# sylvainma/Summarizer

Measured on AMD Instinct MI355X. Metric: frames scored/sec (T x 1024), higher is better.
Workload: dtype f32; 1 GPU; vasnet score, S-TVSum: 50 videos/GPU, T~U(150,320) (sum 12003), D=1024, packed batch; parallelism=video-sharded x1

## Files before the change

summarizer_amd/csrc/gemm_device.h:

```cpp
#pragma once
#include "sumk_internal.h"

namespace sumk {

typedef float f32x16 __attribute__((ext_vector_type(16)));
typedef float f32x4 __attribute__((ext_vector_type(4)));

struct GemmKArgs {
  const float* A;
  const float* B[4];
  float* C;
  const float* R;
  const float* bias0[4];
  const float* bias1[4];
  const GemmProb* probs;
  int32_t nprob;
  int32_t n_group;
  int32_t total_tiles;
  Drop drop; uint32_t drop_site;
  int32_t xcd_tiles_m;
  int32_t group_remap;
  float alpha;
  int32_t lean;
  float* moments;
  unsigned short* C16;
  const float* ln_stats; const float* ln_c1; const float* ln_c2;
  int32_t sk_epi; float* sk_part; unsigned* sk_cnt; float* Csel[4];
};

typedef const __attribute__((address_space(4))) int64_t* cptr64;
typedef const __attribute__((address_space(4))) int32_t* cptr32;
__device__ __forceinline__ int prob_tile_start(const GemmProb* p, int i) { return ((cptr32)(uintptr_t)(p + i))[15]; }
__device__ __forceinline__ GemmProb load_prob(const GemmProb* p, int i) {
  const cptr64 q = (cptr64)(uintptr_t)(p + i);
  const cptr32 r = (cptr32)(uintptr_t)(p + i);
  GemmProb P;
  P.a_off = q[0]; P.b_off = q[1]; P.c_off = q[2]; P.r_off = q[3];
  P.M = r[8]; P.N = r[9]; P.K = r[10]; P.lda = r[11]; P.ldb = r[12]; P.ldc = r[13]; P.ldr = r[14];
  P.tile_start = r[15]; P.tiles_n = r[16];
  return P;
}
static_assert(offsetof(GemmProb, M) == 32 && offsetof(GemmProb, tile_start) == 60 && offsetof(GemmProb, tiles_n) == 64, "GemmProb layout");

struct TileCtx {
  int64_t c_off, r_off;
  int32_t M, N, K, lda, ldb, ldc, ldr, m0, n0, klast;
  const float* ab; const float* bb;
};

template <int BM, int BN>
// ... 90 lines not shown
          if (ka.drop.thr) v = drop_apply(ka.drop, ka.drop_site, (uint64_t)row * (uint64_t)cur.N + (uint64_t)col, v);
          v += ka.R[cur.r_off + (int64_t)row * cur.ldr + col];
        }
        if constexpr (EPI == EPI_ACCUM) v = *cp + ka.alpha * v;
        if constexpr (EPI == EPI_NONE) {
          if (ka.C) *cp = v;
          if (ka.C16) ka.C16[cur.c_off + (int64_t)row * cur.ldc + col] = __builtin_bit_cast(unsigned short, (__bf16)v);
        } else {
          *cp = v;
        }
      }
    }
  }
}

__device__ __forceinline__ float dpp_row_sum16(float v) {
  v += __builtin_bit_cast(float, __builtin_amdgcn_update_dpp(0, __builtin_bit_cast(int, v), 0xB1, 0xF, 0xF, true));
  v += __builtin_bit_cast(float, __builtin_amdgcn_update_dpp(0, __builtin_bit_cast(int, v), 0x4E, 0xF, 0xF, true));
  v += __builtin_bit_cast(float, __builtin_amdgcn_update_dpp(0, __builtin_bit_cast(int, v), 0x141, 0xF, 0xF, true));
  v += __builtin_bit_cast(float, __builtin_amdgcn_update_dpp(0, __builtin_bit_cast(int, v), 0x140, 0xF, 0xF, true));
  return v;
}

template <int TM, int TN>
__device__ __forceinline__ void epilogue_head_moments(const GemmKArgs& ka, const TileCtx& cur, const f32x16 (&acc)[TM][TN], int row0,
                                                      int col0, int li, int lh, float2* lds_stats, int m0, int tid) {
  static_assert(TN == 2, "head epilogue: a wave covers one 64-column slot");
  float bias[TN], gw[TN], c1[TN];
  bool colok[TN];
  const bool ln = ka.ln_stats != nullptr;
  if (ln) {
    __syncthreads();
    if (tid < 128) lds_stats[tid] = reinterpret_cast<const float2*>(ka.ln_stats)[min(m0 + tid, cur.M - 1)];
    __syncthreads();
  }
#pragma unroll
  for (int tn = 0; tn < TN; ++tn) {
    const int col = col0 + tn * 32 + li;
    colok[tn] = col < cur.N;
    const int cc = colok[tn] ? col : 0;
    bias[tn] = ka.bias0[0][cc];
    gw[tn] = ka.bias1[0][cc] * ka.bias1[1][cc];
    c1[tn] = 0.f;
    if (ln) { c1[tn] = ka.ln_c1[cc]; bias[tn] += ka.ln_c2[cc]; }
  }
  const int slots = cur.N >> 5, slot = (col0 >> 5) + (li >> 4);
  float4* part = reinterpret_cast<float4*>(ka.C);
#pragma unroll
  for (int tm = 0; tm < TM; ++tm) {
#pragma unroll
    for (int r = 0; r < 16; ++r) {
      float s1 = 0.f, s2 = 0.f, s3 = 0.f;
      float mean = 0.f, rstd = 1.f;
      if (ln) {
        const float2 st = lds_stats[row0 - m0 + tm * 32 + (r & 3) + 8 * (r >> 2) + 4 * lh];
        mean = st.x; rstd = st.y;
      }
#pragma unroll
      for (int tn = 0; tn < TN; ++tn) {
        float v = rstd * (acc[tm][tn][r] - mean * c1[tn]) + bias[tn];
        v = (v < 0.f) ? 0.f : v;
        if (!colok[tn]) v = 0.f;
        s1 += v; s2 += v * v; s3 += v * gw[tn];
      }
      s1 = dpp_row_sum16(s1); s2 = dpp_row_sum16(s2); s3 = dpp_row_sum16(s3);
      const int row = row0 + tm * 32 + (r & 3) + 8 * (r >> 2) + 4 * lh;
      if ((li & 15) == 0 && row < cur.M) part[(int64_t)row * slots + slot] = make_float4(s1, s2, s3, 0.f);
    }
  }
}

template <int TM, int TN>
__device__ __forceinline__ void epilogue_row_moments(const GemmKArgs& ka, const TileCtx& cur, const f32x16 (&acc)[TM][TN], int row0,
                                                     int col0, int li, int lh) {
  static_assert(TN == 1 || TN == 2, "moments epilogue: a wave covers 32 or 64 columns");
  bool colok[TN];
#pragma unroll
  for (int tn = 0; tn < TN; ++tn) colok[tn] = col0 + tn * 32 + li < cur.N;
  const int slots = TN == 2 ? cur.N >> 5 : cur.N >> 4, slot = (TN == 2 ? col0 >> 5 : col0 >> 4) + (li >> 4);
  float2* part = reinterpret_cast<float2*>(ka.moments) + (cur.c_off / cur.ldc) * slots;
#pragma unroll
  for (int tm = 0; tm < TM; ++tm) {
#pragma unroll
    for (int r = 0; r < 16; ++r) {
      float s1 = 0.f, s2 = 0.f;
#pragma unroll
      for (int tn = 0; tn < TN; ++tn) {
        const float v = colok[tn] ? acc[tm][tn][r] : 0.f;
        s1 += v; s2 += v * v;
      }
      s1 = dpp_row_sum16(s1); s2 = dpp_row_sum16(s2);
      const int row = row0 + tm * 32 + (r & 3) + 8 * (r >> 2) + 4 * lh;
      if ((li & 15) == 0 && row < cur.M) part[(int64_t)row * slots + slot] = make_float2(s1, s2);
    }
// ... 26 lines not shown
```

summarizer_amd/csrc/gemm_f32.hip:

```cpp
#include "gemm_regstage.h"

namespace sumk {

int launch_gemm(GemmLayout layout, GemmEpi epi, const GemmLaunch& g, hipStream_t stream) {
  SUMK_ARG(g.A && g.B[0] && (g.C || (g.C16 && epi == EPI_NONE)) && g.probs, "gemm: null operand");
  if (g.total_tiles <= 0) return SUMK_OK;
  GemmKArgs ka;
  ka.A = g.A;
  for (int i = 0; i < 4; ++i) { ka.B[i] = g.B[i]; ka.bias0[i] = g.bias0[i]; ka.bias1[i] = g.bias1[i]; }
  ka.C = g.C; ka.R = g.R; ka.probs = g.probs; ka.nprob = g.nprob; ka.n_group = g.n_group; ka.alpha = g.alpha;
  ka.total_tiles = g.total_tiles; ka.xcd_tiles_m = 0;
  const bool small_groups = (int64_t)g.total_tiles <= (int64_t)256 * g.nprob;
  ka.group_remap = (g.nprob > 1 && (g.group_remap || (g.precision != SUMK_PRECISION_FP32 && small_groups))) ? 1 : 0;
  ka.drop.seed = g.drop_seed; ka.drop.thr = g.drop_thr; ka.drop.scale = g.drop_scale; ka.drop.seed_dev = nullptr; ka.drop_site = g.drop_site;
  ka.lean = (g.lean && g.nprob == 1 && layout == GEMM_NT && g.small_tile == 0 && g.precision == SUMK_PRECISION_FP32 &&
             (g.n_group == 0 || g.n_group % 128 == 0)) ? 1 : 0;
  ka.C16 = (unsigned short*)g.C16;
  SUMK_ARG(!g.C16 || epi == EPI_NONE, "gemm: the bf16 copy of C goes with the plain epilogue");
  SUMK_ARG(!g.src16 || (g.small_tile == 0 && g.n_group == 0), "gemm: bf16-source launches use 128x128 tiles and one B operand");
  ka.moments = g.moments; ka.ln_stats = g.ln_stats; ka.ln_c1 = g.ln_c1; ka.ln_c2 = g.ln_c2;
  SUMK_ARG(epi != EPI_RESIDUAL_MOMENTS || g.moments, "gemm: the moments epilogue needs an output buffer");
  SUMK_ARG(!g.ln_stats || (epi == EPI_BIAS_RELU_HEAD && g.ln_c1 && g.ln_c2), "gemm: ln_stats goes with the head epilogue and c1 / c2");
  if (g.prof_tag >= 0) prof_begin(g.prof_tag, stream);
  prof_begin(SUMK_PROF_GEMM_ALL, stream);
  if (g.nprob == 1 && g.xcd_M > 0) {
    const int bm = (g.src16 && g.wide16) ? g.wide16 : gemm_tile_m(g.small_tile), bn = (g.src16 && g.wide16) ? 256 : gemm_tile_n(g.small_tile);
    const int tm = (g.xcd_M + bm - 1) / bm, tn = (g.xcd_N + bn - 1) / bn;
    if (tn % 4 == 0 && tm >= 16) { ka.xcd_tiles_m = tm; ka.total_tiles = 8 * ((tm + 1) / 2) * (tn / 4); }
  }
  int rc;
  ka.sk_epi = (int32_t)epi; ka.sk_part = g.sk_part; ka.sk_cnt = g.sk_cnt;
  for (int i = 0; i < 4; ++i) ka.Csel[i] = g.Csel[i];
  if (g.sk) {
    SUMK_ARG(g.precision == SUMK_PRECISION_FP32 && g.small_tile == 1 && g.n_group == 0 && !g.src16 && !g.C16 && g.C,
             "gemm: an SK launch is exact fp32 on 64x64 tiles with one B group per table entry");
    SUMK_ARG(epi == EPI_NONE || epi == EPI_RESIDUAL || epi == EPI_BIAS_RELU || epi == EPI_ACCUM, "gemm: epilogue %d has no SK form", (int)epi);
    SUMK_ARG(g.drop_thr == 0, "gemm: SK launches have no epilogue dropout");
    ka.group_remap = 0; ka.xcd_tiles_m = 0;
    rc = launch_gemm_lean(layout, ka, ka.total_tiles, stream, 1);
    prof_end(SUMK_PROF_GEMM_ALL, stream);
    if (g.prof_tag >= 0) prof_end(g.prof_tag, stream);
    if (rc != SUMK_OK) return rc;
    SUMK_HIP(hipGetLastError());
    return SUMK_OK;
  }
// ... 356 lines not shown
```

summarizer_amd/csrc/gemm_regstage.h:

```cpp
#pragma once
#include "gemm_device.h"
#include <algorithm>
#include <cstdlib>

namespace sumk {

typedef __bf16 bf16x4 __attribute__((ext_vector_type(4)));
typedef __bf16 bf16x8 __attribute__((ext_vector_type(8)));
typedef short s16x4 __attribute__((ext_vector_type(4)));
typedef short s16x8 __attribute__((ext_vector_type(8)));

__device__ __forceinline__ float4 ldg4(const float* p) { return *reinterpret_cast<const float4*>(p); }

__device__ __forceinline__ bf16x8 tr_frag(const char* p, int pitch) {
  typedef __attribute__((address_space(3))) s16x4* lds_s16x4;
  const s16x4 h0 = __builtin_amdgcn_ds_read_tr16_b64_v4i16((lds_s16x4)(p));
  const s16x4 h1 = __builtin_amdgcn_ds_read_tr16_b64_v4i16((lds_s16x4)(p + 4 * pitch));
  return __builtin_bit_cast(bf16x8, __builtin_shufflevector(h0, h1, 0, 1, 2, 3, 4, 5, 6, 7));
}

template <int BM, int BN, int BK, bool A_KC, bool B_KC, int EPI, int NS = 0, bool LEAN = false>
__global__ __launch_bounds__(256, 3) void gemm_f32_kernel(GemmKArgs ka) {
  static_assert(!LEAN || (A_KC && B_KC && NS == 0), "LEAN: NT fp32 instances only");
  constexpr bool X3 = NS > 0;
  static_assert(NS >= 0 && NS <= 3, "operand split: 0 (fp32), 1 (plain bf16), 2 or 3 bf16 planes");
  constexpr int KC_PITCH = (NS == 0 ? BK : NS * BK / 2) + 4;
  constexpr int TPK = BK / 4, RPP = 256 / TPK;
  constexpr int WTM = BM / 2, WTN = BN / 2;
  constexpr int TM = WTM / 32, TN = WTN / 32;
  constexpr int NLDA = BM * BK / 1024, NLDB = BN * BK / 1024;
  constexpr int MCP_A = 2 * BM + 64, MCP_B = 2 * BN + 64;
  constexpr int A_ELEMS = A_KC ? BM * KC_PITCH : (X3 ? NS * BK * MCP_A / 4 : BK * BM);
  constexpr int B_ELEMS = B_KC ? BN * KC_PITCH : (X3 ? NS * BK * MCP_B / 4 : BK * BN);
  constexpr int STAGE = A_ELEMS + B_ELEMS;
  __shared__ __attribute__((aligned(16))) float lds[STAGE];
  float* sA = lds;
  float* sB = lds + A_ELEMS;

  const int tid = threadIdx.x;
  const int lane = tid & 63;
  const int wave = tid >> 6;
  const int wm = wave >> 1, wn = wave & 1;
  const int li = lane & 31, lh = lane >> 5;
  constexpr int TPRA = BM / 4, TPRB = BN / 4;
  constexpr int KROWSA = 256 / TPRA, KROWSB = 256 / TPRB;
  const int kq4 = (tid % TPK) * 4;

  const float* pa[NLDA];
  const float* pb[NLDB];
  int voa[NLDA], vob[NLDB];

  auto setup = [&](int tile, TileCtx& c) -> bool {
    GemmProb P;
    if (!decode_tile<BM, BN>(ka, tile, c, P)) return false;
    if constexpr (LEAN) {
      c.ab = ka.A + P.a_off;
      int g = 0, ng = 0;
      if (ka.n_group > 0) { g = c.n0 / ka.n_group; ng = g * ka.n_group; }
// ... 201 lines not shown
            float4 v = *reinterpret_cast<const float4*>(&sB[(wn * WTN + t * 32 + li) * KC_PITCH + kk * 8 + 4 * lh]);
            bv[t][0] = v.x; bv[t][1] = v.y; bv[t][2] = v.z; bv[t][3] = v.w;
          } else {
#pragma unroll
            for (int j = 0; j < 4; ++j) bv[t][j] = sB[(kk * 8 + 4 * lh + j) * BN + wn * WTN + t * 32 + li];
          }
        }
#pragma unroll
        for (int j = 0; j < 4; ++j)
#pragma unroll
          for (int tm = 0; tm < TM; ++tm)
#pragma unroll
            for (int tn = 0; tn < TN; ++tn)
              acc[tm][tn] = __builtin_amdgcn_mfma_f32_32x32x2f32(av[tm][j], bv[tn][j], acc[tm][tn], 0, 0, 0);
      }
      }
  };

  int tile = blockIdx.x;
  if (tile >= ka.total_tiles) return;
  TileCtx cur, nxt;
  if (!setup(tile, cur)) return;
  gload(cur, 0);

  while (true) {
    f32x16 acc[TM][TN];
    if constexpr (EPI == EPI_RESIDUAL || EPI == EPI_RESIDUAL_MOMENTS) {
      residual_init<TM, TN>(ka, cur, acc, cur.m0 + wm * WTM, cur.n0 + wn * WTN, li, lh);
    } else {
#pragma unroll
      for (int i = 0; i < TM; ++i)
#pragma unroll
        for (int j = 0; j < TN; ++j)
#pragma unroll
          for (int r = 0; r < 16; ++r) acc[i][j][r] = 0.f;
    }

    const int next_tile = tile + gridDim.x;
    bool has_next = false;
    const int K = cur.K;
    {
      int k0 = 0;
      for (; k0 + BK < K; k0 += BK) {
        __syncthreads();
        swrite(sA, sB);
        __syncthreads();
        gload(cur, k0 + BK);
        compute(sA, sB, acc);
      }
      __syncthreads();
      ktail(K, k0);
      swrite(sA, sB);
      __syncthreads();
      has_next = next_tile < ka.total_tiles;
      if (has_next) has_next = setup(next_tile, nxt);
      if (has_next) gload(nxt, 0);
      compute(sA, sB, acc);
    }

    if constexpr (EPI == EPI_BIAS_RELU_HEAD) {
      epilogue_head_moments<TM, TN>(ka, cur, acc, cur.m0 + wm * WTM, cur.n0 + wn * WTN, li, lh, reinterpret_cast<float2*>(lds), cur.m0, tid);
    } else if constexpr (EPI == EPI_RESIDUAL_MOMENTS) {
      epilogue_row_moments<TM, TN>(ka, cur, acc, cur.m0 + wm * WTM, cur.n0 + wn * WTN, li, lh);
      epilogue_store<EPI, TM, TN, true>(ka, cur, acc, cur.m0 + wm * WTM, cur.n0 + wn * WTN, li, lh);
    } else {
      epilogue_store<EPI, TM, TN, true>(ka, cur, acc, cur.m0 + wm * WTM, cur.n0 + wn * WTN, li, lh);
    }
    if (!has_next) break;
    tile = next_tile;
    cur = nxt;
  }
}

template <int BM, int BN, int BK, bool A_KC, bool B_KC, int X3 = 0>
static int launch_epi(GemmEpi epi, const GemmKArgs& ka, int tiles, hipStream_t s) {
  constexpr int occ = (BM == 128 && BN == 128) ? 3 : (BM == 128 ? 4 : (BK == 64 ? 4 : 8));
  dim3 grid(std::min(tiles, 256 * occ)), block(256);
  if constexpr (BM == 128 && BN == 128 && BK == 32 && A_KC && B_KC && X3 == 0) {
    if (ka.lean) {
#define SUMK_LEAN_CASE(E) case E: hipLaunchKernelGGL((gemm_f32_kernel<BM, BN, BK, true, true, E, 0, true>), grid, block, 0, s, ka); return SUMK_OK;
      switch (epi) {
        SUMK_LEAN_CASE(EPI_NONE) SUMK_LEAN_CASE(EPI_RESIDUAL) SUMK_LEAN_CASE(EPI_BIAS_RELU) SUMK_LEAN_CASE(EPI_BIAS2)
        SUMK_LEAN_CASE(EPI_BIAS_RESIDUAL) SUMK_LEAN_CASE(EPI_BIAS_RELU_HEAD) SUMK_LEAN_CASE(EPI_RESIDUAL_MOMENTS)
        default: break;
      }
#undef SUMK_LEAN_CASE
    }
  }
  switch (epi) {
    case EPI_NONE: hipLaunchKernelGGL((gemm_f32_kernel<BM, BN, BK, A_KC, B_KC, EPI_NONE, X3>), grid, block, 0, s, ka); break;
    case EPI_RESIDUAL: hipLaunchKernelGGL((gemm_f32_kernel<BM, BN, BK, A_KC, B_KC, EPI_RESIDUAL, X3>), grid, block, 0, s, ka); break;
    case EPI_BIAS_RELU: hipLaunchKernelGGL((gemm_f32_kernel<BM, BN, BK, A_KC, B_KC, EPI_BIAS_RELU, X3>), grid, block, 0, s, ka); break;
    case EPI_BIAS2: hipLaunchKernelGGL((gemm_f32_kernel<BM, BN, BK, A_KC, B_KC, EPI_BIAS2, X3>), grid, block, 0, s, ka); break;
    case EPI_ACCUM: hipLaunchKernelGGL((gemm_f32_kernel<BM, BN, BK, A_KC, B_KC, EPI_ACCUM, X3>), grid, block, 0, s, ka); break;
    case EPI_BIAS_RESIDUAL: hipLaunchKernelGGL((gemm_f32_kernel<BM, BN, BK, A_KC, B_KC, EPI_BIAS_RESIDUAL, X3>), grid, block, 0, s, ka); break;
    case EPI_BIAS_RELU_HEAD:
      if constexpr (BM == 128 && BN == 128 && BK == 32 && A_KC && B_KC) {
        hipLaunchKernelGGL((gemm_f32_kernel<BM, BN, BK, A_KC, B_KC, EPI_BIAS_RELU_HEAD, X3>), grid, block, 0, s, ka); break;
      } else { set_error("gemm: the head epilogue exists for 128x128 NT tiles only"); return SUMK_ERR_ARG; }
    case EPI_RESIDUAL_MOMENTS:
      if constexpr ((BM == 128 && BN == 128 && BK == 32 && A_KC && B_KC) || (BM == 64 && BN == 64 && BK == 32 && A_KC && !B_KC)) {
        hipLaunchKernelGGL((gemm_f32_kernel<BM, BN, BK, A_KC, B_KC, EPI_RESIDUAL_MOMENTS, X3>), grid, block, 0, s, ka); break;
      } else { set_error("gemm: the moments epilogue exists for 128x128 NT and 64x64 NN tiles only"); return SUMK_ERR_ARG; }
    default: set_error("gemm: bad epilogue %d", (int)epi); return SUMK_ERR_ARG;
  }
  return SUMK_OK;
}

template <int BM, int BN, int BK, int X3 = 0>
static int launch_layout(GemmLayout layout, GemmEpi epi, const GemmKArgs& ka, int tiles, hipStream_t s) {
  if (layout == GEMM_NT) return launch_epi<BM, BN, BK, true, true, X3>(epi, ka, tiles, s);
  if (layout == GEMM_NN) return launch_epi<BM, BN, BK, true, false, X3>(epi, ka, tiles, s);
  return launch_epi<BM, BN, BK, false, false, X3>(epi, ka, tiles, s);
}


}
```

summarizer_amd/csrc/sumk_internal.h:

```cpp
#pragma once
#include <hip/hip_runtime.h>
#include <stdint.h>
#include <stddef.h>
#include "../../include/sumk.h"

namespace sumk {

void set_error(const char* fmt, ...);
int hip_fail(hipError_t e, const char* what);

#define SUMK_HIP(call)                                             \
  do {                                                             \
    hipError_t _e = (call);                                        \
    if (_e != hipSuccess) return ::sumk::hip_fail(_e, #call);      \
  } while (0)
#define SUMK_ARG(cond, ...)                                        \
  do {                                                             \
    if (!(cond)) { ::sumk::set_error(__VA_ARGS__); return SUMK_ERR_ARG; } \
  } while (0)
#define SUMK_TRY(call)                                             \
  do { int _r = (call); if (_r != SUMK_OK) return _r; } while (0)

inline size_t align_up(size_t v, size_t a) { return (v + a - 1) / a * a; }


struct GemmProb {
  int64_t a_off, b_off, c_off, r_off;
  int32_t M, N, K;
  int32_t lda, ldb, ldc, ldr;
  int32_t tile_start;
  int32_t tiles_n;
  int32_t pad_[7];
};
static_assert(sizeof(GemmProb) == 96, "GemmProb layout");
enum { SK_N = 0, SK_IDX = 1, SK_TILE0 = 2, SK_BSEL = 3, SK_CSEL = 4, SK_PART0 = 5 };

enum GemmLayout { GEMM_NT = 0, GEMM_NN = 1, GEMM_TN = 2 };
enum GemmEpi {
  EPI_NONE = 0,
  EPI_RESIDUAL = 1,
  EPI_BIAS_RELU = 2,
  EPI_BIAS2 = 3,
  EPI_ACCUM = 4,
  EPI_BIAS_RESIDUAL = 5,
  EPI_BIAS_RELU_HEAD = 6,
  EPI_RESIDUAL_MOMENTS = 7,
};

struct GemmLaunch {
  const float* A = nullptr;
  const float* B[4] = {nullptr, nullptr, nullptr, nullptr};
  float* C = nullptr;
  const float* R = nullptr;
  const float* bias0[4] = {nullptr, nullptr, nullptr, nullptr};
  const float* bias1[4] = {nullptr, nullptr, nullptr, nullptr};
  const GemmProb* probs = nullptr;
  int32_t nprob = 1;
  int32_t n_group = 0;
  int32_t total_tiles = 0;
  float alpha = 1.f;
  int32_t small_tile = 0;
  int32_t prof_tag = -1;
  int32_t precision = 0;
  int32_t xcd_M = 0, xcd_N = 0;
  int32_t no_dma = 0;
  uint64_t drop_seed = 0; uint32_t drop_thr = 0, drop_site = 0; float drop_scale = 1.f;
  float* moments = nullptr;
  int32_t lean = 0;
  int32_t src16 = 0;
  int32_t wide16 = 0;
  void* C16 = nullptr;
  int32_t group_remap = 0;
  const float* ln_stats = nullptr; const float* ln_c1 = nullptr; const float* ln_c2 = nullptr;
  int32_t sk = 0; float* sk_part = nullptr; unsigned* sk_cnt = nullptr; float* Csel[4] = {nullptr, nullptr, nullptr, nullptr};
};
constexpr int SK_MAX_SLICES = 8;
inline int sk_slices(int tiles, int K, int* kchunk) {
  int S = tiles > 0 ? 1024 / tiles : 1;
  S = S < 1 ? 1 : S > SK_MAX_SLICES ? SK_MAX_SLICES : S;
  if (S > K / 128) S = K / 128 < 1 ? 1 : K / 128;
  int kc = ((K + S - 1) / S + 31) / 32 * 32;
  S = (K + kc - 1) / kc;
  *kchunk = kc;
  return S;
}

inline int gemm_tile_m(int cfg) { return cfg == 1 ? 64 : 128; }
inline int gemm_tile_n(int cfg) { return cfg == 0 ? 128 : cfg == 3 ? 256 : 64; }
inline int gemm_tile_dim(int cfg) { return gemm_tile_n(cfg); }
inline int gemm_tiles(int M, int N, int cfg) {
  int tm = gemm_tile_m(cfg), tn = gemm_tile_n(cfg);
  return ((M + tm - 1) / tm) * ((N + tn - 1) / tn);
}
int launch_gemm(GemmLayout layout, GemmEpi epi, const GemmLaunch& g, hipStream_t stream);
inline int gemm_b16_ok(int64_t M, int64_t N, int64_t K, int lda, int ldb, bool kc_a, bool kc_b) {
  const int64_t lim = (int64_t)1 << 31;
// ... 165 lines not shown
```

summarizer_amd/csrc/vasnet.hip:

```cpp
#include "gemm_device.h"
#include <math.h>
#include <algorithm>
#include <cstdlib>

namespace sumk {

enum { TB_S = 0, TB_PV = 1, TB_DV = 2, TB_DP = 3, TB_DQ = 4, TB_DK = 5, TB_COUNT = 6 };
constexpr int ROW_PROBS = 8;
constexpr int SPLITK_PROBS = 64;
constexpr int COLSUM_CHUNKS = 128;

struct VasnetWs {
  size_t qkv, e, ctx, y0, y1, z, seq, prob_row, prob_seq, prob_dvk, prob_skw, stats, scores, row_seq, total;
  size_t total_core;
  size_t e2, dz, dy1, dy0, dctx, dqkv, lnpart, colpart, slab, prob_sk;
  size_t x16, w16, ctx16, y116, dz16, dy016, dqkv16, qkv16, dctx16, p16, s16;
  size_t slab_elems;
  int64_t e_elems;
  int32_t n_rows;
  size_t sk_part, sk_cnt, sk_tabs, sk_part_bytes;
  size_t tab_bytes;
};

constexpr int SK_MAX_ROWS = 1024;
// ... 699 lines not shown
    for (int k = sub; k < slots; k += 8) { const float2 p = moments[(int64_t)row * slots + k]; s1 += p.x; s2 += p.y; }
#pragma unroll
  for (int m = 1; m <= 4; m <<= 1) { s1 += __shfl_xor(s1, m, 64); s2 += __shfl_xor(s2, m, 64); }
  if (row >= n_rows || sub != 0) return;
  const double mean = s1 / D, var = s2 / D - mean * mean;
  stats[row] = make_float2((float)mean, (float)(1.0 / sqrt((var > 0.0 ? var : 0.0) + (double)eps)));
}
__global__ void head_vectors_kernel(const float* __restrict__ b1, const float* __restrict__ c2, const float* __restrict__ ln_w,
                                    const float* __restrict__ w2, int D, float* __restrict__ biasc, float* __restrict__ gw) {
  const int n = blockIdx.x * blockDim.x + threadIdx.x;
  if (n < D) { biasc[n] = b1[n] + c2[n]; gw[n] = ln_w[n] * w2[n]; }
}

struct WPlanes { size_t wqkv, wo, w1g, c1, biasc, gw, tmp, total; };
static WPlanes wplanes_layout(int D, int np) {
  WPlanes l; size_t p = 0;
  auto take = [&](size_t bytes) { size_t at = p; p += align_up(bytes, 256); return at; };
  l.wqkv = take(pw_planes_bytes(3 * (int64_t)D, D, np)); l.wo = take(pw_planes_bytes(D, D, np)); l.w1g = take(pw_planes_bytes(D, D, np));
  l.c1 = take((size_t)D * 4); l.biasc = take((size_t)D * 4); l.gw = take((size_t)D * 4);
  l.tmp = take((size_t)D * D * 4 + (size_t)D * 4);
  l.total = p;
  return l;
}
struct PwExtra { size_t qkv, ap, ctx, total; };
static PwExtra pw_extra(int D, int64_t R, int t_max, int np, size_t base) {
  PwExtra e; size_t p = align_up(base, 256);
  auto take = [&](size_t bytes) { size_t at = p; p += align_up(bytes, 256); return at; };
  e.qkv = take(pw_planes_bytes(R, 3 * D, np)); e.ap = take(pw_alpha_bytes(R, t_max, np)); e.ctx = take(pw_planes_bytes(R, D, np));
  e.total = p;
  return e;
}
constexpr int PW_LONG_TMIN = 1536;
struct PwLong { size_t e, qp, kp, vt, ap, st, qk, total; int tn, kpad, qk_direct; };
static PwLong pw_long_layout(int D, int64_t R, int t_max, int np, size_t base) {
  PwLong e; size_t p = align_up(base, 256);
  auto take = [&](size_t bytes) { size_t at = p; p += align_up(bytes, 256); return at; };
  e.tn = (t_max + 255) / 256 * 256; e.kpad = (t_max + 31) / 32 * 32;
  e.e = take((size_t)t_max * e.tn * 4);
  e.qk_direct = (R >= e.tn && pw_ok(R, 2 * (int64_t)D, D, R, 3 * (int64_t)D, np) && (int64_t)pw_planes_bytes(R, 2 * D, np) < (((int64_t)1 << 31) - 65536)) ? 1 : 0;
  e.qk = take(e.qk_direct ? pw_planes_bytes(R, 2 * D, np) : 0);
  e.qp = take(e.qk_direct ? 0 : pw_planes_bytes(e.tn, D, np)); e.kp = take(e.qk_direct ? 0 : pw_planes_bytes(e.tn, D, np));
  e.vt = take(pw_planes_bytes(D, e.kpad, np)); e.ap = take(pw_planes_bytes(t_max, e.kpad, np));
  e.st = take((size_t)t_max * 8);
  e.total = p;
  return e;
}
// ... 419 lines not shown
  float* none[4] = {nullptr, nullptr, nullptr, nullptr};
  SUMK_TRY(gemm_tn_splitk_accum_multi(2, As, Bs, D, D, D, D, R, nullptr, L.slab_elems, pskw, SPLITK_PROBS, none, D, D, 1.f, stream, precision, b16, SPLITK_TABLE_ONLY));
  SUMK_TRY(gemm_tn_splitk_accum((const float*)base, 3 * D, (const float*)base, D, 3 * D, D, R, nullptr, L.slab_elems, pskw + SPLITK_PROBS, SPLITK_PROBS, none, D, D, 1.f,
                                stream, precision, b16, SPLITK_TABLE_ONLY));
  return SUMK_OK;
}

extern "C" int sumk_vasnet_build_tables(int32_t D, int32_t n_seq, const int32_t* seq_off_host, const int32_t* seq_off_dev, int32_t training,
                                        int32_t precision, void* tables, size_t tables_bytes, void* stream_) {
  hipStream_t stream = (hipStream_t)stream_;
  SUMK_ARG(seq_off_dev && tables && ((uintptr_t)tables & 255) == 0, "vasnet_build_tables: null or misaligned (256 B) pointer");
  SUMK_ARG(precision >= SUMK_PRECISION_FP32 && precision <= SUMK_PRECISION_MAX, "vasnet_build_tables: unknown precision %d", precision);
  Geometry G;
  SUMK_TRY(geometry(D, n_seq, seq_off_host, training, precision, 0, &G));
  if (tables_bytes < G.L.tab_bytes) { set_error("vasnet_build_tables: %zu bytes < required %zu", tables_bytes, G.L.tab_bytes); return SUMK_ERR_WORKSPACE; }
  launch_setup(G, D, n_seq, seq_off_dev, (char*)tables, stream);
  if (G.sk) SUMK_TRY(launch_sk_setup(G, D, n_seq, seq_off_dev, (char*)tables, stream));
  if (training) SUMK_TRY(build_skw_tables(G, D, (GemmProb*)((char*)tables + G.L.prob_skw), precision, stream));
  SUMK_HIP(hipGetLastError());
  return SUMK_OK;
}

extern "C" size_t sumk_vasnet_wplanes_bytes(int32_t D, int32_t n_planes) {
  return wplanes_ok(D, n_planes) ? wplanes_layout(D, n_planes).total : 0;
}

extern "C" int sumk_vasnet_wplanes_build(int32_t D, const sumk_vasnet_weights* w, const float* Wvo, int32_t n_planes, void* out, size_t out_bytes,
                                         void* stream_) {
  hipStream_t stream = (hipStream_t)stream_;
  SUMK_ARG(wplanes_ok(D, n_planes), "vasnet_wplanes_build: D=%d planes=%d is not eligible (D %% 256, 2 or 3 planes)", D, n_planes);
  SUMK_ARG(w && w->Wk && w->Wq && w->Wv && w->Wo && w->W1 && w->b1 && w->w2 && w->ln_w && w->ln_b && out, "vasnet_wplanes_build: null pointer");
  const WPlanes l = wplanes_layout(D, n_planes);
  SUMK_ARG(out_bytes >= l.total && ((uintptr_t)out & 255) == 0, "vasnet_wplanes_build: buffer of %zu bytes (256-byte aligned) needed, got %zu", l.total, out_bytes);
  char* o = (char*)out;
  SUMK_HIP(hipMemsetAsync(o, 0, l.c1, stream));
  const float* parts[3] = {w->Wq, w->Wk, Wvo ? Wvo : w->Wv};
  for (int i = 0; i < 3; ++i) SUMK_TRY(split_planes_at(parts[i], D, D, D, n_planes, o + l.wqkv, (int64_t)i * D, 3 * (int64_t)D, stream));
  SUMK_TRY(split_planes(w->Wo, D, D, D, n_planes, o + l.wo, stream));
  float* W1g = (float*)(o + l.tmp); float* c2 = W1g + (size_t)D * D;
  hipLaunchKernelGGL(ln_fold_stats_kernel, dim3(D), dim3(256), 0, stream, w->W1, w->ln_w, w->ln_b, D, W1g, (float*)(o + l.c1), c2,
                     (const float2*)nullptr, 0, 0, 0.f, (float2*)nullptr);
  SUMK_HIP(hipGetLastError());
  SUMK_TRY(split_planes(W1g, D, D, D, n_planes, o + l.w1g, stream));
  hipLaunchKernelGGL(head_vectors_kernel, dim3((D + 255) / 256), dim3(256), 0, stream, w->b1, c2, w->ln_w, w->w2, D, (float*)(o + l.biasc), (float*)(o + l.gw));
  SUMK_HIP(hipGetLastError());
  return SUMK_OK;
}

extern "C" size_t sumk_vasnet_workspace_bytes(int32_t D, int32_t n_seq, const int32_t* seq_off_host, int32_t training) {
  VasnetWs w;
  if (carve(D, n_seq, seq_off_host, training, &w) != SUMK_OK) return 0;
  return w.total;
// ... 236 lines not shown
    const dim3 sg((R + 3) / 4), sb(256);
    float* e2p = use_e2 ? E2 : nullptr;
    unsigned short* p16 = b16 ? (unsigned short*)(ws + L.p16) : nullptr;
#define SUMK_SOFTMAX(NR) hipLaunchKernelGGL(vasnet_softmax_kernel<NR>, sg, sb, 0, stream, E, e2p, seq, (const int32_t*)(tb + L.row_seq), n_seq, R, opts->scale, opts->ignore_self, opts->aperture, drop, p16, (const float*)E, 0, (int64_t)0)
    if (t_max <= 256) SUMK_SOFTMAX(4); else if (t_max <= 512) SUMK_SOFTMAX(8); else if (t_max <= 1024) SUMK_SOFTMAX(16); else SUMK_SOFTMAX(0);
#undef SUMK_SOFTMAX
  }
  }
  static const bool fused_head_on = !(getenv("SUMK_FUSED_HEAD") && getenv("SUMK_FUSED_HEAD")[0] == '0');
  static const bool fused_ln_on = !(getenv("SUMK_FUSED_LN") && getenv("SUMK_FUSED_LN")[0] == '0');
  const bool fused_tail = fused_head_on && !training && drop.thr == 0 && G.st_d == 0 && D % 64 == 0;
  const int ln_slots = Wvo ? D / 16 : D / 32;
  const size_t ln_mom_f = align_up((size_t)R * ln_slots * 2, 64), ln_w_f = (size_t)D * D, ln_c_f = align_up((size_t)2 * D, 64);
  const bool fused_ln = pw || (fused_tail && fused_ln_on && (!Wvo || G.cfg_pv == 1) && ln_mom_f + ln_w_f + ln_c_f + (size_t)2 * R <= (size_t)R * D);
  char* const pw_ctxp = pw_attn ? ws + px.ctx : ws + L.y0;
  char* const pw_y0p = (pw_attn && Wvo) ? ws + px.ctx : pw_attn ? ws + px.qkv : ws + L.qkv;
  float* const pw_mom = Z;
  float* const pw_stats = Z + align_up((size_t)R * (D / 16) * 2, 64);
  float* const pw_part = pw_stats + align_up((size_t)R * 2, 64);
  float* ln_moments = pw ? pw_mom : Y1;
  float* ln_W1g = Y1 + ln_mom_f;
  float* ln_c1 = ln_W1g + ln_w_f;
  float* ln_stats = ln_c1 + ln_c_f;
  if (!G.attn_fused && !pw_attn && !pw_long) {
    GemmLaunch g; g.precision = opts->precision;
    g.A = use_e2 ? E2 : E; g.B[0] = QKV; g.C = Wvo ? Y0 : CTX; g.R = x; g.probs = tabs + TB_PV * n_seq; g.nprob = n_seq; g.small_tile = G.cfg_pv;
    g.total_tiles = G.tiles_pv; g.prof_tag = SUMK_PROF_GEMM_PV;
    if (Wvo && fused_ln) g.moments = ln_moments;
    if (b16) { g.A = (const float*)(ws + L.p16); g.B[0] = (const float*)(ws + L.qkv16); g.src16 = 1; g.C16 = ws + L.ctx16; g.C = nullptr; }
    SUMK_TRY(launch_gemm(GEMM_NN, Wvo ? (fused_ln ? EPI_RESIDUAL_MOMENTS : EPI_RESIDUAL) : EPI_NONE, g, stream));
    if (Wvo && pw) {
      hipLaunchKernelGGL(ln_row_stats_kernel, dim3((R + 31) / 32), dim3(256), 0, stream, (const float2*)pw_mom, ln_slots, R, D, opts->eps, (float2*)pw_stats);
      SUMK_HIP(hipGetLastError());
      SUMK_TRY(split_planes(Y0, R, D, D, np, pw_y0p, stream));
    } else
    if (Wvo && fused_ln) {
      hipLaunchKernelGGL(ln_fold_stats_kernel, dim3(D + (R + 31) / 32), dim3(256), 0, stream, w->W1, w->ln_w, w->ln_b, D, ln_W1g, ln_c1,
                         ln_c1 + D, (const float2*)ln_moments, ln_slots, R, opts->eps, (float2*)ln_stats);
      SUMK_HIP(hipGetLastError());
    }
  }
  if (pw_attn && Wvo) {
    hipLaunchKernelGGL(ln_row_stats_kernel, dim3((R + 31) / 32), dim3(256), 0, stream, (const float2*)pw_mom, D / 32, R, D, opts->eps, (float2*)pw_stats);
    SUMK_HIP(hipGetLastError());
  } else
  if (pw && !Wvo) {
    if (!pw_attn && !pw_long) SUMK_TRY(split_planes(CTX, R, D, D, np, pw_ctxp, stream));
    PwLaunch g; g.A = pw_ctxp; g.a_rows = R; g.B = wp + wl.wo; g.b_rows = D; g.M = R; g.N = D; g.K = D; g.np = np;
    g.R = x; g.ldr = D; g.moments = pw_mom; g.O = pw_y0p; g.o_rows = R; g.prof_tag = SUMK_PROF_GEMM_OPROJ;
    SUMK_TRY(launch_gemm_pw(PW_RES_MOM_PLANES, g, stream));
    hipLaunchKernelGGL(ln_row_stats_kernel, dim3((R + 31) / 32), dim3(256), 0, stream, (const float2*)pw_mom, D / 64, R, D, opts->eps, (float2*)pw_stats);
    SUMK_HIP(hipGetLastError());
  } else
  if (!Wvo) {
    GemmLaunch g; g.precision = opts->precision;
    g.A = CTX; g.B[0] = w->Wo; g.C = Y0; g.R = x; g.probs = prow + RP_DD; g.small_tile = G.st_d;
    g.total_tiles = gemm_tiles(R, D, G.st_d); g.xcd_M = R; g.xcd_N = D; g.prof_tag = SUMK_PROF_GEMM_OPROJ;
    g.lean = lean_rows;
    if (fused_ln) {
      g.moments = ln_moments;
      SUMK_TRY(launch_gemm(GEMM_NT, EPI_RESIDUAL_MOMENTS, g, stream));
      hipLaunchKernelGGL(ln_fold_stats_kernel, dim3(D + (R + 31) / 32), dim3(256), 0, stream, w->W1, w->ln_w, w->ln_b, D, ln_W1g, ln_c1,
                         ln_c1 + D, (const float2*)ln_moments, ln_slots, R, opts->eps, (float2*)ln_stats);
      SUMK_HIP(hipGetLastError());
    } else {
      if (b16) to_b16(g, ws + L.ctx16, Wo16, R, D, prow, RP_DD_W);
      SUMK_TRY(launch_gemm(GEMM_NT, EPI_RESIDUAL, g, stream));
    }
  }
  if (!fused_ln) launch_ln_rows<false>(Y0, b16 ? nullptr : Y1, w->ln_w, w->ln_b, nullptr, nullptr, nullptr, R, D, opts->eps, stats, drop, 1u, stream,
                                       b16 ? (unsigned short*)(ws + L.y116) : nullptr);
  if (pw) {
    PwLaunch g; g.A = pw_y0p; g.a_rows = R; g.B = wp + wl.w1g; g.b_rows = D; g.M = R; g.N = D; g.K = D; g.np = np;
    g.bias = (const float*)(wp + wl.biasc); g.gw = (const float*)(wp + wl.gw); g.ln_c1 = (const float*)(wp + wl.c1); g.ln_stats = pw_stats;
    g.head_part = pw_part; g.prof_tag = SUMK_PROF_GEMM_K1;
    SUMK_TRY(launch_gemm_pw(PW_HEAD, g, stream));
    hipLaunchKernelGGL(head_finalize_kernel, dim3((R + 31) / 32), dim3(256), 0, stream, (const float4*)pw_part, D / 64, R, D, w->ln_w,
                       w->ln_b, w->w2, w->b2, opts->eps, scores);
    SUMK_HIP(hipGetLastError());
    return SUMK_OK;
  }
  if (fused_tail) {
    GemmLaunch g; g.precision = opts->precision;
    g.A = Y1; g.B[0] = w->W1; g.bias0[0] = w->b1; g.bias1[0] = w->ln_w; g.bias1[1] = w->w2;
    if (fused_ln) { g.A = Y0; g.B[0] = ln_W1g; g.ln_stats = ln_stats; g.ln_c1 = ln_c1; g.ln_c2 = ln_c1 + D; }
    g.C = Z;
    g.probs = prow + RP_DD; g.small_tile = 0;
    g.total_tiles = gemm_tiles(R, D, 0); g.xcd_M = R; g.xcd_N = D; g.prof_tag = SUMK_PROF_GEMM_K1;
    g.lean = lean_rows;
    SUMK_TRY(launch_gemm(GEMM_NT, EPI_BIAS_RELU_HEAD, g, stream));
    hipLaunchKernelGGL(head_finalize_kernel, dim3((R + 31) / 32), dim3(256), 0, stream, (const float4*)Z, D / 32, R, D, w->ln_w,
                       w->ln_b, w->w2, w->b2, opts->eps, scores);
    SUMK_HIP(hipGetLastError());
    return SUMK_OK;
  }
  {
    GemmLaunch g; g.precision = opts->precision;
    g.A = Y1; g.B[0] = w->W1; g.bias0[0] = w->b1; g.C = Z; g.probs = prow + RP_DD; g.small_tile = G.st_d;
    g.total_tiles = gemm_tiles(R, D, G.st_d); g.xcd_M = R; g.xcd_N = D; g.prof_tag = SUMK_PROF_GEMM_K1;
    g.lean = lean_rows;
    if (b16) to_b16(g, ws + L.y116, W116, R, D, prow, RP_DD_W);
    SUMK_TRY(launch_gemm(GEMM_NT, EPI_BIAS_RELU, g, stream));
  }
  launch_ln_rows<true>(Z, training ? (float*)(ws + L.scores) : nullptr, w->ln_w, w->ln_b, w->w2, w->b2, scores, R, D, opts->eps, stats ? stats + 2 * (size_t)R : nullptr, drop, 2u, stream);
  SUMK_HIP(hipGetLastError());
  return SUMK_OK;
}

extern "C" int sumk_vasnet_forward(float* x, int32_t D, int32_t n_seq, const int32_t* seq_off_host,
                                   const int32_t* seq_off_dev, const sumk_vasnet_weights* w,
                                   const sumk_vasnet_opts* opts, const float* pos_table, const int32_t* pos_rows,
                                   float* scores, void* workspace, size_t workspace_bytes, int32_t training,
                                   void* stream) {
// ... 240 lines not shown
```

summarizer_amd/models/vasnet.py:

```python
import math
import random
import numpy as np
import torch
import torch.nn as nn
import torch.nn.init as init

from .. import kernels
from ..autograd import SegmentMseMeanFunction
from . import Trainer
from ._positional import PositionalInput, _sinusoid_table, packed_pos_input
from ..training import FlatAdam, dist_info, plan_shards, resolve_batch_videos, step_video_total


class VASNet(PositionalInput, nn.Module):
    def __init__(self, input_size=1024, max_length=None, pos_embed="simple", ignore_self=False,
                 attention_aperture=None, scale=None, epsilon=1e-6, weight_init="xavier", precision="fp32", fold_vo=False):
        super().__init__()
        self.precision = precision
        self.fold_vo = bool(fold_vo)
        self._wvo, self._wvo_key = None, None
        self.input_size = input_size
        self.aperture = attention_aperture
        self.ignore_self = ignore_self
        self.scale = scale if scale is not None else 1 / np.sqrt(self.input_size)
# ... 43 lines not shown

    def score_packed(self, x_packed, lens):
        sb = kernels.SeqBatch.get(lens, x_packed.device)
        if self.max_length is None:
            return self._score(x_packed, sb, None, None)
        plane_path = self.precision in kernels.PLANES_OF and self.input_size % 256 == 0 and sb.n_rows >= 256
        xp, extra = packed_pos_input(self, x_packed, sb, self.precision, kernels.PLANES_OF[self.precision] if plane_path else 0)
        return self._score(xp, sb, None, None, extra)

    def _score(self, xp, sb, table, rows, extra=None):
        training = self.training and torch.is_grad_enabled()
        if training or (torch.is_grad_enabled() and any(p.requires_grad for p in self.parameters())):
            from ..autograd import VasnetFunction
            names = [k for _, k in kernels.VASNET_FIELDS]
            p = self._params()
            opts = self._opts(self.training)
            opts.update(extra or {})
            return VasnetFunction.apply(xp, sb, opts, table, rows, names, *[p[n] for n in names])
        opts = self._opts(False)
        opts.update(extra or {})
        wvo = self._folded() if self.fold_vo else None
        if self.precision in kernels.PLANES_OF and table is None and self.input_size % 256 == 0 and sb.n_rows >= 256:
            opts["wplanes"] = self._wplanes(wvo)
        scores, _ = kernels.vasnet_forward_packed(xp, sb, self._params(), opts, table, rows, training=False, wvo=wvo)
        return scores

    def _wplanes(self, wvo):
        p = self._params()
        key = kernels.weights_key([v for _, v in sorted(p.items())], self.precision, bool(self.fold_vo))
        return kernels.cached_block(self, "_wpl", key, lambda out: kernels.vasnet_wplanes(
            {k: v.detach() for k, v in p.items()}, self.input_size, kernels.PLANES_OF[self.precision], wvo=wvo, out=out))

    def _folded(self):
        wo, wv = self.attention_head_projection.weight, self.V.weight
        key = (wo.data_ptr(), wv.data_ptr(), wo._version, wv._version, kernels.WEIGHTS_EPOCH[0])
        if self._wvo is None or self._wvo_key != key:
            with torch.no_grad():
                self._wvo = kernels.fold_vo(wo.detach(), wv.detach(), out=self._wvo if self._wvo is not None and self._wvo.device == wo.device else None)
            self._wvo_key = key
        return self._wvo

    def _drop_weight_caches(self):
        self._wvo_key = None
        self._wpl_key = None

    def invalidate_folded(self):
        self._drop_weight_caches()

    def train(self, mode=True):
        self._drop_weight_caches()
        return super().train(mode)

    def load_state_dict(self, *args, **kwargs):
        self._drop_weight_caches()
# ... 127 lines not shown
```

Measured before the change: 10.49 million frames/s.

## Compute LN row statistics inside the head GEMM and cache the folded W1 weights

Adds a head epilogue variant where each 128x128 tile reduces the per-row moment partials into mean and rstd in shared memory, using double accumulation, right after its first loads are issued. This removes the separate ln_fold_stats launch for fp32 inference. The gamma-folded W1 and the c1/c2 vectors are now built once into a cached weights block keyed on weight versions, so they are no longer recomputed on every forward. In exchange, each column tile re-reads the row moments redundantly, adds two extra barriers per tile, and needs more LDS.

```diff
diff --git a/summarizer_amd/csrc/gemm_device.h b/summarizer_amd/csrc/gemm_device.h
--- a/summarizer_amd/csrc/gemm_device.h
+++ b/summarizer_amd/csrc/gemm_device.h
@@ -26,6 +26,7 @@
   unsigned short* C16;
   const float* ln_stats; const float* ln_c1; const float* ln_c2;
   int32_t sk_epi; float* sk_part; unsigned* sk_cnt; float* Csel[4];
+  const float* ln_moments_in; int32_t ln_slots; float ln_eps;
 };
 
 typedef const __attribute__((address_space(4))) int64_t* cptr64;
@@ -162,14 +163,14 @@
   return v;
 }
 
-template <int TM, int TN>
+template <int TM, int TN, bool STATS_READY = false>
 __device__ __forceinline__ void epilogue_head_moments(const GemmKArgs& ka, const TileCtx& cur, const f32x16 (&acc)[TM][TN], int row0,
                                                       int col0, int li, int lh, float2* lds_stats, int m0, int tid) {
   static_assert(TN == 2, "head epilogue: a wave covers one 64-column slot");
   float bias[TN], gw[TN], c1[TN];
   bool colok[TN];
-  const bool ln = ka.ln_stats != nullptr;
-  if (ln) {
+  const bool ln = STATS_READY || ka.ln_stats != nullptr;
+  if (ln && !STATS_READY) {
     __syncthreads();
     if (tid < 128) lds_stats[tid] = reinterpret_cast<const float2*>(ka.ln_stats)[min(m0 + tid, cur.M - 1)];
     __syncthreads();
@@ -210,6 +211,51 @@
   }
 }
 
+__device__ __forceinline__ void head_row_stats(const GemmKArgs& ka, const TileCtx& cur, float* lds, float2* lds_stats, int tid) {
+  const float2* mom = reinterpret_cast<const float2*>(ka.ln_moments_in);
+  int K = cur.K; float eps = ka.ln_eps;
+  asm volatile("" : "+v"(tid), "+s"(K), "+s"(eps));
+  const int slots = ka.ln_slots, sub = tid & 7, rl0 = tid >> 3;
+  double* sums = reinterpret_cast<double*>(lds);
+  __syncthreads();
+  constexpr int NK = 4;
+  if (slots <= 8 * NK) {
+    float2 q[4][NK];
+#pragma unroll
+    for (int p = 0; p < 4; ++p) {
+      const int row = min(cur.m0 + p * 32 + rl0, cur.M - 1);
+#pragma unroll
+      for (int u = 0; u < NK; ++u) q[p][u] = sub + 8 * u < slots ? mom[(int64_t)row * slots + sub + 8 * u] : make_float2(0.f, 0.f);
+    }
+#pragma unroll
+    for (int p = 0; p < 4; ++p) {
+      double s1 = 0.0, s2 = 0.0;
+#pragma unroll
+      for (int u = 0; u < NK; ++u)
+        if (sub + 8 * u < slots) { s1 += q[p][u].x; s2 += q[p][u].y; }
+#pragma unroll
+      for (int m = 1; m <= 4; m <<= 1) { s1 += __shfl_xor(s1, m, 64); s2 += __shfl_xor(s2, m, 64); }
+      if (sub == 0) { sums[2 * (p * 32 + rl0)] = s1; sums[2 * (p * 32 + rl0) + 1] = s2; }
+    }
+  } else {
+#pragma unroll 1
+    for (int p = 0; p < 4; ++p) {
+      const int row = min(cur.m0 + p * 32 + rl0, cur.M - 1);
+      double s1 = 0.0, s2 = 0.0;
+      for (int k = sub; k < slots; k += 8) { const float2 q = mom[(int64_t)row * slots + k]; s1 += q.x; s2 += q.y; }
+#pragma unroll
+      for (int m = 1; m <= 4; m <<= 1) { s1 += __shfl_xor(s1, m, 64); s2 += __shfl_xor(s2, m, 64); }
+      if (sub == 0) { sums[2 * (p * 32 + rl0)] = s1; sums[2 * (p * 32 + rl0) + 1] = s2; }
+    }
+  }
+  __syncthreads();
+  if (tid < 128) {
+    const double s1 = sums[2 * tid], s2 = sums[2 * tid + 1];
+    const double mean = s1 / K, var = s2 / K - mean * mean;
+    lds_stats[tid] = make_float2((float)mean, (float)(1.0 / sqrt((var > 0.0 ? var : 0.0) + (double)eps)));
+  }
+}
+
 template <int TM, int TN>
 __device__ __forceinline__ void epilogue_row_moments(const GemmKArgs& ka, const TileCtx& cur, const f32x16 (&acc)[TM][TN], int row0,
                                                      int col0, int li, int lh) {
diff --git a/summarizer_amd/csrc/gemm_f32.hip b/summarizer_amd/csrc/gemm_f32.hip
--- a/summarizer_amd/csrc/gemm_f32.hip
+++ b/summarizer_amd/csrc/gemm_f32.hip
@@ -21,6 +21,9 @@
   ka.moments = g.moments; ka.ln_stats = g.ln_stats; ka.ln_c1 = g.ln_c1; ka.ln_c2 = g.ln_c2;
   SUMK_ARG(epi != EPI_RESIDUAL_MOMENTS || g.moments, "gemm: the moments epilogue needs an output buffer");
   SUMK_ARG(!g.ln_stats || (epi == EPI_BIAS_RELU_HEAD && g.ln_c1 && g.ln_c2), "gemm: ln_stats goes with the head epilogue and c1 / c2");
+  ka.ln_moments_in = g.ln_moments_in; ka.ln_slots = g.ln_slots; ka.ln_eps = g.ln_eps;
+  SUMK_ARG(epi != EPI_BIAS_RELU_HEAD_ROWS || (g.ln_moments_in && g.ln_slots > 0 && g.ln_c1 && g.ln_c2 && ka.lean && !g.src16 && !g.sk),
+           "gemm: the head epilogue with in-launch row statistics is one exact-fp32 NT problem on the buffer-load 128x128 instance, with moments and c1 / c2");
   if (g.prof_tag >= 0) prof_begin(g.prof_tag, stream);
   prof_begin(SUMK_PROF_GEMM_ALL, stream);
   if (g.nprob == 1 && g.xcd_M > 0) {
diff --git a/summarizer_amd/csrc/gemm_regstage.h b/summarizer_amd/csrc/gemm_regstage.h
--- a/summarizer_amd/csrc/gemm_regstage.h
+++ b/summarizer_amd/csrc/gemm_regstage.h
@@ -33,7 +33,9 @@
   constexpr int A_ELEMS = A_KC ? BM * KC_PITCH : (X3 ? NS * BK * MCP_A / 4 : BK * BM);
   constexpr int B_ELEMS = B_KC ? BN * KC_PITCH : (X3 ? NS * BK * MCP_B / 4 : BK * BN);
   constexpr int STAGE = A_ELEMS + B_ELEMS;
-  __shared__ __attribute__((aligned(16))) float lds[STAGE];
+  constexpr bool HEAD_ROWS = EPI == EPI_BIAS_RELU_HEAD_ROWS;
+  static_assert(!HEAD_ROWS || (BM == 128 && BN == 128 && A_KC && B_KC && NS == 0 && LEAN), "in-launch row statistics: the exact-fp32 buffer-load instance on 128x128 NT tiles");
+  __shared__ __attribute__((aligned(16))) float lds[STAGE + (HEAD_ROWS ? 256 : 0)];
   float* sA = lds;
   float* sB = lds + A_ELEMS;
 
@@ -281,6 +283,7 @@
   TileCtx cur, nxt;
   if (!setup(tile, cur)) return;
   gload(cur, 0);
+  if constexpr (HEAD_ROWS) head_row_stats(ka, cur, lds, reinterpret_cast<float2*>(lds + STAGE), tid);
 
   while (true) {
     f32x16 acc[TM][TN];
@@ -317,7 +320,9 @@
       compute(sA, sB, acc);
     }
 
-    if constexpr (EPI == EPI_BIAS_RELU_HEAD) {
+    if constexpr (HEAD_ROWS) {
+      epilogue_head_moments<TM, TN, true>(ka, cur, acc, cur.m0 + wm * WTM, cur.n0 + wn * WTN, li, lh, reinterpret_cast<float2*>(lds + STAGE), cur.m0, tid);
+    } else if constexpr (EPI == EPI_BIAS_RELU_HEAD) {
       epilogue_head_moments<TM, TN>(ka, cur, acc, cur.m0 + wm * WTM, cur.n0 + wn * WTN, li, lh, reinterpret_cast<float2*>(lds), cur.m0, tid);
     } else if constexpr (EPI == EPI_RESIDUAL_MOMENTS) {
       epilogue_row_moments<TM, TN>(ka, cur, acc, cur.m0 + wm * WTM, cur.n0 + wn * WTN, li, lh);
@@ -328,6 +333,7 @@
     if (!has_next) break;
     tile = next_tile;
     cur = nxt;
+    if constexpr (HEAD_ROWS) head_row_stats(ka, cur, lds, reinterpret_cast<float2*>(lds + STAGE), tid);
   }
 }
 
@@ -341,6 +347,7 @@
       switch (epi) {
         SUMK_LEAN_CASE(EPI_NONE) SUMK_LEAN_CASE(EPI_RESIDUAL) SUMK_LEAN_CASE(EPI_BIAS_RELU) SUMK_LEAN_CASE(EPI_BIAS2)
         SUMK_LEAN_CASE(EPI_BIAS_RESIDUAL) SUMK_LEAN_CASE(EPI_BIAS_RELU_HEAD) SUMK_LEAN_CASE(EPI_RESIDUAL_MOMENTS)
+        SUMK_LEAN_CASE(EPI_BIAS_RELU_HEAD_ROWS)
         default: break;
       }
 #undef SUMK_LEAN_CASE
@@ -357,6 +364,7 @@
       if constexpr (BM == 128 && BN == 128 && BK == 32 && A_KC && B_KC) {
         hipLaunchKernelGGL((gemm_f32_kernel<BM, BN, BK, A_KC, B_KC, EPI_BIAS_RELU_HEAD, X3>), grid, block, 0, s, ka); break;
       } else { set_error("gemm: the head epilogue exists for 128x128 NT tiles only"); return SUMK_ERR_ARG; }
+    case EPI_BIAS_RELU_HEAD_ROWS: set_error("gemm: the head epilogue with in-launch row statistics needs GemmLaunch::lean (exact fp32, 128x128 NT tiles, K %% 32 == 0)"); return SUMK_ERR_ARG;
     case EPI_RESIDUAL_MOMENTS:
       if constexpr ((BM == 128 && BN == 128 && BK == 32 && A_KC && B_KC) || (BM == 64 && BN == 64 && BK == 32 && A_KC && !B_KC)) {
         hipLaunchKernelGGL((gemm_f32_kernel<BM, BN, BK, A_KC, B_KC, EPI_RESIDUAL_MOMENTS, X3>), grid, block, 0, s, ka); break;
diff --git a/summarizer_amd/csrc/sumk_internal.h b/summarizer_amd/csrc/sumk_internal.h
--- a/summarizer_amd/csrc/sumk_internal.h
+++ b/summarizer_amd/csrc/sumk_internal.h
@@ -45,6 +45,7 @@
   EPI_BIAS_RESIDUAL = 5,
   EPI_BIAS_RELU_HEAD = 6,
   EPI_RESIDUAL_MOMENTS = 7,
+  EPI_BIAS_RELU_HEAD_ROWS = 8,
 };
 
 struct GemmLaunch {
@@ -72,6 +73,7 @@
   void* C16 = nullptr;
   int32_t group_remap = 0;
   const float* ln_stats = nullptr; const float* ln_c1 = nullptr; const float* ln_c2 = nullptr;
+  const float* ln_moments_in = nullptr; int32_t ln_slots = 0; float ln_eps = 0.f;
   int32_t sk = 0; float* sk_part = nullptr; unsigned* sk_cnt = nullptr; float* Csel[4] = {nullptr, nullptr, nullptr, nullptr};
 };
 constexpr int SK_MAX_SLICES = 8;
diff --git a/summarizer_amd/csrc/vasnet.hip b/summarizer_amd/csrc/vasnet.hip
--- a/summarizer_amd/csrc/vasnet.hip
+++ b/summarizer_amd/csrc/vasnet.hip
@@ -745,6 +745,15 @@
   l.total = p;
   return l;
 }
+struct WFold { size_t w1g, c1, c2, total; };
+static bool wfold_ok(int D) { return D > 0 && D % 4 == 0; }
+static WFold wfold_layout(int D) {
+  WFold l; size_t p = 0;
+  auto take = [&](size_t bytes) { size_t at = p; p += align_up(bytes, 256); return at; };
+  l.w1g = take((size_t)D * D * 4); l.c1 = take((size_t)D * 4); l.c2 = take((size_t)D * 4);
+  l.total = p;
+  return l;
+}
 struct PwExtra { size_t qkv, ap, ctx, total; };
 static PwExtra pw_extra(int D, int64_t R, int t_max, int np, size_t base) {
   PwExtra e; size_t p = align_up(base, 256);
@@ -1210,12 +1219,24 @@
 }
 
 extern "C" size_t sumk_vasnet_wplanes_bytes(int32_t D, int32_t n_planes) {
+  if (n_planes == 0) return wfold_ok(D) ? wfold_layout(D).total : 0;
   return wplanes_ok(D, n_planes) ? wplanes_layout(D, n_planes).total : 0;
 }
 
 extern "C" int sumk_vasnet_wplanes_build(int32_t D, const sumk_vasnet_weights* w, const float* Wvo, int32_t n_planes, void* out, size_t out_bytes,
                                          void* stream_) {
   hipStream_t stream = (hipStream_t)stream_;
+  if (n_planes == 0) {
+    SUMK_ARG(wfold_ok(D), "vasnet_wplanes_build: D=%d is not eligible (D %% 4)", D);
+    SUMK_ARG(w && w->W1 && w->ln_w && w->ln_b && out, "vasnet_wplanes_build: null pointer");
+    const WFold f = wfold_layout(D);
+    SUMK_ARG(out_bytes >= f.total && ((uintptr_t)out & 255) == 0, "vasnet_wplanes_build: buffer of %zu bytes (256-byte aligned) needed, got %zu", f.total, out_bytes);
+    char* o = (char*)out;
+    hipLaunchKernelGGL(ln_fold_stats_kernel, dim3(D), dim3(256), 0, stream, w->W1, w->ln_w, w->ln_b, D, (float*)(o + f.w1g), (float*)(o + f.c1),
+                       (float*)(o + f.c2), (const float2*)nullptr, 0, 0, 0.f, (float2*)nullptr);
+    SUMK_HIP(hipGetLastError());
+    return SUMK_OK;
+  }
   SUMK_ARG(wplanes_ok(D, n_planes), "vasnet_wplanes_build: D=%d planes=%d is not eligible (D %% 256, 2 or 3 planes)", D, n_planes);
   SUMK_ARG(w && w->Wk && w->Wq && w->Wv && w->Wo && w->W1 && w->b1 && w->w2 && w->ln_w && w->ln_b && out, "vasnet_wplanes_build: null pointer");
   const WPlanes l = wplanes_layout(D, n_planes);
@@ -1498,6 +1519,15 @@
   float* ln_W1g = Y1 + ln_mom_f;
   float* ln_c1 = ln_W1g + ln_w_f;
   float* ln_stats = ln_c1 + ln_c_f;
+  static const bool fused_rows_on = !(getenv("SUMK_FUSED_ROWS") && getenv("SUMK_FUSED_ROWS")[0] == '0');
+  const bool rows_in_k1 = fused_rows_on && fused_tail && fused_ln && !Wvo && !pw && !b16 && opts->precision == SUMK_PRECISION_FP32 && lean_rows &&
+                          D % 128 == 0 && opts->wplanes != nullptr && wfold_ok(D);
+  if (rows_in_k1) {
+    const WFold wf = wfold_layout(D);
+    SUMK_ARG(((uintptr_t)opts->wplanes & 255) == 0, "vasnet_forward: opts->wplanes must be 256-byte aligned");
+    ln_W1g = (float*)((char*)opts->wplanes + wf.w1g); ln_c1 = (float*)((char*)opts->wplanes + wf.c1);
+  }
+  const float* const ln_c2 = rows_in_k1 ? (const float*)((const char*)opts->wplanes + wfold_layout(D).c2) : ln_c1 + D;
   if (!G.attn_fused && !pw_attn && !pw_long) {
     GemmLaunch g; g.precision = opts->precision;
     g.A = use_e2 ? E2 : E; g.B[0] = QKV; g.C = Wvo ? Y0 : CTX; g.R = x; g.probs = tabs + TB_PV * n_seq; g.nprob = n_seq; g.small_tile = G.cfg_pv;
@@ -1536,9 +1566,11 @@
     if (fused_ln) {
       g.moments = ln_moments;
       SUMK_TRY(launch_gemm(GEMM_NT, EPI_RESIDUAL_MOMENTS, g, stream));
-      hipLaunchKernelGGL(ln_fold_stats_kernel, dim3(D + (R + 31) / 32), dim3(256), 0, stream, w->W1, w->ln_w, w->ln_b, D, ln_W1g, ln_c1,
-                         ln_c1 + D, (const float2*)ln_moments, ln_slots, R, opts->eps, (float2*)ln_stats);
-      SUMK_HIP(hipGetLastError());
+      if (!rows_in_k1) {
+        hipLaunchKernelGGL(ln_fold_stats_kernel, dim3(D + (R + 31) / 32), dim3(256), 0, stream, w->W1, w->ln_w, w->ln_b, D, ln_W1g, ln_c1,
+                           ln_c1 + D, (const float2*)ln_moments, ln_slots, R, opts->eps, (float2*)ln_stats);
+        SUMK_HIP(hipGetLastError());
+      }
     } else {
       if (b16) to_b16(g, ws + L.ctx16, Wo16, R, D, prow, RP_DD_W);
       SUMK_TRY(launch_gemm(GEMM_NT, EPI_RESIDUAL, g, stream));
@@ -1559,12 +1591,13 @@
   if (fused_tail) {
     GemmLaunch g; g.precision = opts->precision;
     g.A = Y1; g.B[0] = w->W1; g.bias0[0] = w->b1; g.bias1[0] = w->ln_w; g.bias1[1] = w->w2;
-    if (fused_ln) { g.A = Y0; g.B[0] = ln_W1g; g.ln_stats = ln_stats; g.ln_c1 = ln_c1; g.ln_c2 = ln_c1 + D; }
+    if (fused_ln) { g.A = Y0; g.B[0] = ln_W1g; g.ln_stats = ln_stats; g.ln_c1 = ln_c1; g.ln_c2 = ln_c2; }
+    if (rows_in_k1) { g.ln_stats = nullptr; g.ln_moments_in = ln_moments; g.ln_slots = ln_slots; g.ln_eps = opts->eps; }
     g.C = Z;
     g.probs = prow + RP_DD; g.small_tile = 0;
     g.total_tiles = gemm_tiles(R, D, 0); g.xcd_M = R; g.xcd_N = D; g.prof_tag = SUMK_PROF_GEMM_K1;
     g.lean = lean_rows;
-    SUMK_TRY(launch_gemm(GEMM_NT, EPI_BIAS_RELU_HEAD, g, stream));
+    SUMK_TRY(launch_gemm(GEMM_NT, rows_in_k1 ? EPI_BIAS_RELU_HEAD_ROWS : EPI_BIAS_RELU_HEAD, g, stream));
     hipLaunchKernelGGL(head_finalize_kernel, dim3((R + 31) / 32), dim3(256), 0, stream, (const float4*)Z, D / 32, R, D, w->ln_w,
                        w->ln_b, w->w2, w->b2, opts->eps, scores);
     SUMK_HIP(hipGetLastError());
diff --git a/summarizer_amd/models/vasnet.py b/summarizer_amd/models/vasnet.py
--- a/summarizer_amd/models/vasnet.py
+++ b/summarizer_amd/models/vasnet.py
@@ -89,14 +89,18 @@
         wvo = self._folded() if self.fold_vo else None
         if self.precision in kernels.PLANES_OF and table is None and self.input_size % 256 == 0 and sb.n_rows >= 256:
             opts["wplanes"] = self._wplanes(wvo)
+        elif (kernels.precision_code(self.precision) == 0 and wvo is None and self.input_size % 128 == 0 and xp.is_cuda
+              and -(-sb.n_rows // 128) * (self.input_size // 128) >= 512 and not torch.cuda.is_current_stream_capturing()):
+            opts["wplanes"] = self._wplanes(None, 0)
         scores, _ = kernels.vasnet_forward_packed(xp, sb, self._params(), opts, table, rows, training=False, wvo=wvo)
         return scores
 
-    def _wplanes(self, wvo):
+    def _wplanes(self, wvo, n_planes=None):
         p = self._params()
+        n_planes = kernels.PLANES_OF[self.precision] if n_planes is None else n_planes
         key = kernels.weights_key([v for _, v in sorted(p.items())], self.precision, bool(self.fold_vo))
         return kernels.cached_block(self, "_wpl", key, lambda out: kernels.vasnet_wplanes(
-            {k: v.detach() for k, v in p.items()}, self.input_size, kernels.PLANES_OF[self.precision], wvo=wvo, out=out))
+            {k: v.detach() for k, v in p.items()}, self.input_size, n_planes, wvo=wvo, out=out))
 
     def _folded(self):
         wo, wv = self.attention_head_projection.weight, self.V.weight
```

Result: no change. 10.42 million frames/s (-0.6%).
